# jrnerupudinho/Semi-Blind-Channel-Estimation-for-MIMO-RIS-communication-system-Using-EM-Algo

Measured on AMD Instinct MI355X. Metric: EM-iterations/sec (whole node) + NMSE@SNR; Nt=Nr=4, N_RIS=64, Tp=16 Td=256, higher is better.
Workload: dtype f64; 1 GPU; cfg1; n_tx=4, n_rx=4, N_RIS=64, T_p=16, T_d=256, M=16, trials_per_gpu=1000, em_iters=20, estep=soft, partition_r=0, solve=chol, parallelism=trials-sharded x1, streams_per_gpu=3

## Files before the change

semi-blind-channel-estimation-for-mimo-ris-communication-system-using-em-algo_amd/csrc/api.hip:

```cpp
#include <stdlib.h>
#include <string.h>

#include <atomic>
#include <initializer_list>
#include <mutex>
#include <vector>

#include "sbce_internal.h"

using namespace sbce;

namespace sbce {

#if SBCE_AB
DebugConfig g_debug;

namespace {
void read_debug_env(DebugConfig& c) {
    c = kDebugDefault;
    auto env = [](const char* n) { const char* v = getenv(n); return (v && v[0]) ? v : nullptr; };
    const char* v;
    if ((v = env("SBCE_ESTEP_IMPL"))) c.estep_valu = v[0] == 'v';
    if ((v = env("SBCE_ESTEP_PRUNE"))) c.estep_noprune = v[0] == '0';
    if ((v = env("SBCE_ESTEP_COUNT"))) c.estep_count = v[0] == '1';
    if ((v = env("SBCE_ESTEP_F32"))) c.estep_nof32 = v[0] == '0';
    if ((v = env("SBCE_ESTEP_SPHERE"))) c.estep_nosphere = v[0] == '0';
    if ((v = env("SBCE_SPHERE_BUDGET"))) {
        const int bu = atoi(v);
        c.sphere_budget = bu < 1 ? 1 : (bu > kBfsPmax ? kBfsPmax : bu);
    }
    if ((v = env("SBCE_BACKSUB"))) c.backsub_general = v[0] == '1';
    if ((v = env("SBCE_CHOL_IMPL"))) c.chol_valu = v[0] == 'v';
    if ((v = env("SBCE_ESTEP_PAIR"))) c.estep_nopair = v[0] == '0';
    if ((v = env("SBCE_CPLX3"))) c.cplx3 = v[0] != '0';
    if ((v = env("SBCE_MSTEP_SMALL"))) {
        c.mstep_nosmall = v[0] == '0';
        c.small_valu = v[0] == 'v';
        c.small_v1 = v[0] == '1';
    }
    if ((v = env("SBCE_PM_IMPL"))) c.pm_impl = (v[0] == 'w' || v[0] == 't' || v[0] == 'q') ? v[0] : 0;
    if ((v = env("SBCE_SMALL_SOLVE"))) c.small_col = v[0] == 'c';
    if ((v = env("SBCE_ESTEP_TRI"))) c.estep_tri = (v[0] >= '0' && v[0] <= '2') ? v[0] - '0' : 1;
    if ((v = env("SBCE_ESTEP_ORDER"))) c.estep_noorder = v[0] == '0';
    if ((v = env("SBCE_SMALL_STOP"))) c.small_stop = (v[0] >= '1' && v[0] <= '4') ? v[0] - '0' : 0;
}

__attribute__((constructor)) void load_debug_env() { read_debug_env(g_debug); }
}

bool debug_nondefault() {
    const DebugConfig& c = g_debug;
    const DebugConfig& d = kDebugDefault;
    return c.estep_valu != d.estep_valu || c.estep_noprune != d.estep_noprune ||
           c.estep_nof32 != d.estep_nof32 || c.estep_tri != d.estep_tri || c.estep_noorder != d.estep_noorder ||
           c.estep_nosphere != d.estep_nosphere || c.sphere_budget != d.sphere_budget ||
           c.backsub_general != d.backsub_general || c.chol_valu != d.chol_valu ||
           c.estep_nopair != d.estep_nopair || c.cplx3 != d.cplx3 ||
           c.mstep_nosmall != d.mstep_nosmall || c.small_stop != d.small_stop ||
           c.small_valu != d.small_valu || c.small_v1 != d.small_v1 || c.small_col != d.small_col ||
           (chol_debug_skip_mask() & 31);
}
#else
bool debug_nondefault() { return false; }
#endif

}

namespace {

constexpr size_t kAlign = 256;
size_t align_up(size_t v) { return (v + kAlign - 1) / kAlign * kAlign; }

struct Carve {
    size_t mom, R, rhs, done, mchg, ysh, prep, list, tree, tol, winv, ppsi, pS, pflag, prhs, gram, grhs,
        act, tol2, dvec, mnr, mnskip, total;
    bool has_prep, has_prhs, has_winv, has_mn;
};

constexpr int kAnySolve = -1;

bool make_problem(const sbce_dims* d, Problem& pb) {
    if (!d) return false;
    if (d->batch < 0 || d->n_tx < 1 || d->n_rx < 1 || d->n_psi < 1 || d->t_p < 0 || d->t_d < 1 ||
        d->m < 2 || d->partition_r < 0 || !(d->varn > 0.0))
        return false;
    if (d->n_tx > 8 || d->n_rx > 8) return false;
    pb.B = d->batch; pb.NT = d->n_tx; pb.NR = d->n_rx; pb.P = d->n_psi;
// ... 777 lines not shown
    Problem pb;
    if (!make_problem(d, pb) || !out3) return SBCE_EINVAL;
    int rc = check_ptrs(p, pb, true, SBCE_SOLVE_MINNORM);
    if (rc) return rc;
    if (pb.B == 0) return SBCE_OK;
    const Carve c = carve(pb, SBCE_SOLVE_MINNORM);
    MstepArgs ma;
    ma.R = (cd*)((char*)p->workspace + c.R);
    ma.done = nullptr;
    ma.nbatch = pb.B;
    set_large(ma, (char*)p->workspace, c);
    return hip_rc(launch_minnorm_rank(pb, ma, out3, (hipStream_t)hip_stream));
}

int sbce_debug_reload_env(void) {
#if SBCE_AB
    read_debug_env(g_debug);
    return debug_nondefault() ? 1 : 0;
#else
    return -1;
#endif
}

int sbce_debug_estep_mfma(unsigned long long* out, int reset) {
    if (!reset && !out) return SBCE_EINVAL;
    return hip_rc(estep_debug_mfma(out, reset));
}

int sbce_debug_estep_groups(unsigned long long* out, int reset) {
    if (!reset && !out) return SBCE_EINVAL;
    return hip_rc(estep_debug_groups(out, reset));
}

int sbce_debug_momskip(unsigned long long* out, int reset) {
#if SBCE_AB
    if (!reset && !out) return SBCE_EINVAL;
    return hip_rc(mstep_debug_momskip(out, reset));
#else
    (void)out; (void)reset;
    return SBCE_EUNSUPPORTED;
#endif
}

int sbce_debug_estep_sphere(unsigned long long* out3, int reset) {
    if (!reset && !out3) return SBCE_EINVAL;
    return hip_rc(estep_debug_sphere(out3, reset));
}

int sbce_debug_estep_pair(unsigned long long* out, int reset) {
    if (!reset && !out) return SBCE_EINVAL;
    return hip_rc(estep_debug_pair(out, reset));
}

int sbce_ser(const sbce_dims* d, const void* x_dest, const void* x_d_true, double* ser_out,
             void* hip_stream) {
    clear_stale_error();
    Problem pb;
    if (!make_problem(d, pb) || !x_dest || !x_d_true || !ser_out) return SBCE_EINVAL;
    if (pb.B == 0) return SBCE_OK;
    return hip_rc(launch_ser(pb, (const cd*)x_dest, (const cd*)x_d_true, ser_out,
                             (hipStream_t)hip_stream));
}

int sbce_gauss_expand(const sbce_dims* d, const void* theta, void* h_out, void* hip_stream) {
    clear_stale_error();
    Problem pb;
// ... 133 lines not shown
```

semi-blind-channel-estimation-for-mimo-ris-communication-system-using-em-algo_amd/csrc/estep_sweep.hip:

```cpp
#include "sbce_internal.h"

namespace sbce {

namespace {


template <int NT, int NR>
__device__ double candidate_distance(const cd* H, const cd* yg, const cd* s_cons, int M,
                                     double reg, cd* scratch, int lane, double& scale) {
    cd* sG = scratch;
    cd* sHy = scratch + 16;
    if (lane < NT * NT) {
        const int u = lane / NT, v = lane - u * NT;
        cd acc = czero();
#pragma unroll
        for (int r = 0; r < NR; ++r) acc = cfmac(acc, H[v * NR + r], H[u * NR + r]);
        if (u == v) acc.x += reg;
        sG[lane] = acc;
    } else if (lane >= 32 && lane < 32 + NT) {
        const int u = lane - 32;
        cd acc = czero();
#pragma unroll
        for (int r = 0; r < NR; ++r) acc = cfmac(acc, yg[r], H[u * NR + r]);
        sHy[u] = acc;
// ... 46 lines not shown
        const double od = shfl_xor_d(bd, off);
        const int os = __shfl_xor(bs, off);
        if (od < bd || (od == bd && os < bs)) { bd = od; bs = os; }
    }
    cd x[NT];
#pragma unroll
    for (int q = 0; q < NT; ++q) x[q] = s_cons[__shfl(bs, 16 * q)];
    double d0 = 0.0, sc = 0.0;
#pragma unroll
    for (int r = 0; r < NR; ++r) {
        cd res = yg[r];
        sc += cabs2(res);
#pragma unroll
        for (int q = 0; q < NT; ++q) {
            const cd hx = cmul(H[q * NR + r], x[q]);
            res = csub(res, hx);
            sc += NT * cabs2(hx);
        }
        d0 += cabs2(res);
    }
    wave_sync();
    scale = sc;
    return d0;
}


constexpr int kMfmaWaves = 2;
constexpr int kChunk = 256;
constexpr int kScreenD = 256;

typedef float f4v __attribute__((ext_vector_type(4)));

constexpr int mfma_rec_d(int rec_words) { return 2 * (rec_words <= 128 ? 160 : (rec_words + 1) / 2 * 2 + 32); }
constexpr int mfma_tri_d(int steps) { return 3 * 64 * steps / 2 + 128; }
constexpr int mfma_tab_d(int NO, int chunk, int steps, int M, int nkt_pad, int rec_words) {
    return (2 * NO + chunk + 3 * (4 * steps) * M + nkt_pad + 128 + 1) / 2 * 2 + mfma_rec_d(rec_words) +
           kScreenD + (M == 16 && chunk == 256 ? mfma_tri_d(steps) : 0);
}
constexpr int kTriGate = 4;

struct MfmaConst {
    int B, Td, P, M, lm;
    int JA, JB, chunk, nparts;
    int tab_d;
    double inv_s2, thr_d;
    double reg;
    int nkt_pad;
    int prune;
    int count;
    int prep_stride;
    int rowb_off;
    int rowb;
    int rec_words;
    int spw;
    int screen;
    int tri;
    int order;
};

template <int NT, int NR>
__device__ double column_tile_bounds(const cd* H, const cd* yg, const cd* s_cons, int M, int lm,
                                     int nkt, double* s_lb, cd* scratch, int lane) {
    constexpr int NA = NT / 2, NB = NT - NA;
    const int mask = M - 1;
    const int r = lane & 7;
    const bool own = r < NR;
    int xa[6];
#pragma unroll
    for (int i = 0; i < 6; ++i) xa[i] = (lane ^ (32 >> i)) << 2;
    auto rsum = [&](double v) {
#pragma unroll
        for (int i = 3; i < 6; ++i) v += bperm_d(v, xa[i]);
        return v;
    };
    auto rdot = [&](cd u, cd v) { return cmk(rsum(fma(v.x, u.x, v.y * u.y)),
                                             rsum(fma(v.y, u.x, -v.x * u.y))); };
    cd u[NA];
    bool ok = true;
#pragma unroll
    for (int q = 0; q < NA; ++q) {
        cd v = own ? H[q * NR + r] : czero();
        const double h2 = rsum(cabs2(v));
#pragma unroll
        for (int rep = 0; rep < 2; ++rep)
#pragma unroll
            for (int j = 0; j < q; ++j) v = csub(v, cmul(u[j], rdot(u[j], v)));
        const double n2 = rsum(cabs2(v));
        ok = ok && h2 > 0.0 && n2 > 1e-6 * h2;
        u[q] = cscale(v, ok ? fast_rsqrt(n2) : 0.0);
// ... 18 lines not shown
#pragma unroll
        for (int b = 0; b < NB; ++b) scratch[8 * (b + 1) + r] = g[b];
    }
    double cmax2 = lane < M ? cabs2(s_cons[lane]) : 0.0;
#pragma unroll
    for (int i = 0; i < 6; ++i) cmax2 = fmax(cmax2, bperm_d(cmax2, xa[i]));
    sc += NB * cmax2 * rsum(g2);
    wave_sync();
    for (int kt0 = 0; kt0 < nkt; kt0 += 4) {
        const int kt = kt0 + (lane >> 4);
        const int k = kt * 16 + (lane & 15);
        cd xb[NB];
#pragma unroll
        for (int b = 0; b < NB; ++b) xb[b] = s_cons[(k >> (lm * (NB - 1 - b))) & mask];
        double lb = 0.0;
#pragma unroll
        for (int rr = 0; rr < NR; ++rr) {
            cd res = scratch[rr];
#pragma unroll
            for (int b = 0; b < NB; ++b) res = csub(res, cmul(scratch[8 * (b + 1) + rr], xb[b]));
            lb += cabs2(res);
        }
        if (!ok) lb = 0.0;
#pragma unroll
        for (int i = 2; i < 6; ++i) lb = fmin(lb, bperm_d(lb, xa[i]));
        if ((lane & 15) == 0 && kt < nkt) s_lb[kt] = lb;
    }
    wave_sync();
    return sc;
}

__device__ unsigned long long g_estep_mfma;
__device__ unsigned long long g_estep_groups;

template <int NT, int NR, int MODE, int TU, bool V16>
__device__ __forceinline__ void estep_mfma_body(const EstepArgs& a, const MfmaConst& c) {
    static_assert(!V16 || NT == 4, "the V16 body is the n_tx = 4, M = 16 sweep");
    const int k_M = V16 ? 16 : c.M;
    const int k_lm = V16 ? 4 : c.lm;
    const int k_JA = V16 ? 256 : c.JA;
    const int k_JB = V16 ? 256 : c.JB;
    const int k_chunk = V16 ? 256 : c.chunk;
    const int k_nkt_pad = V16 ? 16 : c.nkt_pad;
    const int k_rowb_off = V16 ? 4 + 2 * NT * NR + 16 : c.rowb_off;
    const int k_prep_stride = V16 ? k_rowb_off + 6 * NR : c.prep_stride;
    const int k_rec_words = V16 ? k_prep_stride + 2 * NR : c.rec_words;
    const int k_tab_d = V16 ? mfma_tab_d(NT * NR, 256, (2 * NR + 3) / 4, 16, 16, k_rec_words) : c.tab_d;
    constexpr int NA = NT / 2;
    constexpr int NB = NT - NA;
    constexpr int NO = NT * NR;
    constexpr int K2 = 2 * NR;
    constexpr int STEPS = (K2 + 3) / 4;
    constexpr int NPA = NA * (NA - 1) / 2;
    constexpr int NPB = NB * (NB - 1) / 2;
    static_assert(NA >= 1 && NA <= 2 && NB <= 2, "mfma E-step: 2 <= n_tx <= 4");

    if (a.list && (long)blockIdx.x * kMfmaWaves >= (long)a.list[(long)c.B * c.Td]) return;
    extern __shared__ __attribute__((aligned(16))) char smem[];
    cd* s_cons = reinterpret_cast<cd*>(smem);
    const int wave = __builtin_amdgcn_readfirstlane(threadIdx.x >> 6);
    const int lane = threadIdx.x & 63;
    double* wbase = reinterpret_cast<double*>(s_cons + 64) + (size_t)wave * k_tab_d;
    cd* s_heff = reinterpret_cast<cd*>(wbase);
    double* s_al = wbase + 2 * NO;
    double* s_U = s_al + k_chunk;
    double* s_V = s_U + 4 * STEPS * k_M;
    double* s_Q2 = s_V + 4 * STEPS * k_M;
    double* s_lb = s_Q2 + 4 * STEPS * k_M;
    double* s_tab = s_lb + k_nkt_pad;
    double* s_recb = s_tab + 128;
    float* s_al32 = reinterpret_cast<float*>(s_recb + mfma_rec_d(k_rec_words));
    float* s_U32 = s_al32 + 256;

    for (int i = threadIdx.x; i < k_M; i += blockDim.x) s_cons[i] = a.cons[i];
    __syncthreads();

    const long nsym = (long)c.B * c.Td;
    const bool listed = a.list != nullptr;
    int32_t* cnt = listed ? a.list + nsym : nullptr;
    const long nwork = listed ? (long)__builtin_amdgcn_readfirstlane(cnt[0]) : nsym;
    const bool prep = a.prep != nullptr;
    auto sym_of = [&](long gi) -> long { return listed ? (long)a.list[gi] : gi; };
    bool first = true;
    for (;;) {
    long chunk_id;
    if (listed) {
        if (first) {
            chunk_id = (long)blockIdx.x * kMfmaWaves + wave;
        } else {
            int v = 0;
            if (lane == 0) v = atomicAdd(cnt + 1, 1);
            chunk_id = (long)gridDim.x * kMfmaWaves + __builtin_amdgcn_readfirstlane(__shfl(v, 0));
        }
        first = false;
    } else {
        chunk_id = (long)blockIdx.x * kMfmaWaves + wave;
    }
    const int spw = listed ? 1 : c.spw;
    const long g0 = chunk_id * spw;
    if (g0 >= nwork) return;
    const long g1 = g0 + spw < nwork ? g0 + spw : nwork;
    const bool dma = prep && k_rec_words <= 128;
    auto issue = [&](long g, double* dst) {
        int l = lane;
        asm volatile("" : "+v"(l));
        const int hs = k_prep_stride >> 1;
        const double* src = a.prep + (size_t)g * k_prep_stride;
        if (l < hs) src += 2 * l;
        else if (l < (k_rec_words >> 1))
            src = reinterpret_cast<const double*>(a.yd) + (size_t)g * 2 * NR + 2 * (l - hs);
        __builtin_amdgcn_global_load_lds((const __attribute__((address_space(1))) void*)src,
                                         (__attribute__((address_space(3))) void*)dst, 16, 0, 0);
        if (a.done)
            __builtin_amdgcn_global_load_lds(
                (const __attribute__((address_space(1))) void*)(a.done + g / c.Td),
                (__attribute__((address_space(3))) void*)(dst + 128), 4, 0, 0);
    };
    if (dma) issue(sym_of(g0), s_recb);
    for (long gi = g0; gi < g1; ++gi) {
    const long gsym = sym_of(gi);
    const int cur = (int)((gi - g0) & 1);
    double* s_rec = s_recb + cur * 160;
    int dn;
    if (dma) {
        asm volatile("s_waitcnt vmcnt(0)" ::: "memory");
        wave_sync();
        dn = a.done ? reinterpret_cast<const int*>(s_rec + 128)[0] : 0;
        if (gi + 1 < g1) issue(sym_of(gi + 1), s_recb + (cur ^ 1) * 160);
    } else {
        dn = a.done ? a.done[gsym / c.Td] : 0;
        if (prep && !dn) {
            wave_sync();
            for (int e = lane; e < k_rec_words; e += 64)
                s_rec[e] = e < k_prep_stride
                    ? a.prep[(size_t)gsym * k_prep_stride + e]
                    : reinterpret_cast<const double*>(a.yd)[(size_t)gsym * 2 * NR + e - k_prep_stride];
            wave_sync();
        }
    }
    if (dn) continue;
    int lane_s = lane;
    asm volatile("" : "+v"(lane_s));
    [&, lane = lane_s]() {
    const int b = (int)(gsym / c.Td);
    const int t = (int)(gsym - (long)b * c.Td);
    const int mask = k_M - 1;
    double thr_d = c.thr_d, inv_s2 = c.inv_s2, reg = c.reg;
    if (a.varn_t) {
        const TrialNoise tn = trial_noise(a.varn_t[b]);
        thr_d = uniform_d(tn.thr_d);
        inv_s2 = uniform_d(tn.inv_s2);
        reg = uniform_d(tn.reg);
    }

    if (prep) {
    } else {
        const cd* th = a.theta + (size_t)b * c.P * NO;
        const cd* ps = a.psid + (size_t)gsym * c.P;
        const int ntask = NO * c.nparts;
        cd* part = reinterpret_cast<cd*>(s_tab);
        if (lane < ntask) {
// ... 205 lines not shown
#pragma unroll
            for (int j = 0; j < 4; ++j) {
                const double us = bperm_d(uu, (4 * rq + j) << 2);
                tA[(4 * rq + j) * 16 + col] = (float)fma(0.5, (double)cx[j], 0.25 * (us + vv));
            }
            wave_sync();
            double tq = 0.0;
#pragma unroll 1
            for (int blk = 0; blk < 4; ++blk) {
                f4v t[4];
#pragma unroll
                for (int u = 0; u < 4; ++u)
                    t[u] = *reinterpret_cast<const f4v*>(tA + (4 * blk + u) * 16 + rq * 4);
#pragma unroll
                for (int s = 0; s < STEPS; ++s)
#pragma unroll
                    for (int u = 0; u < 4; ++u)
                        t[u] = __builtin_amdgcn_mfma_f32_16x16x4f32(
                            tU[(4 * s + rq) * 16 + 4 * blk + u] + vr32[s], qr32[s], t[u], 0, 0, 0);
                float mm = fminf(fminf(t[0][0], t[0][1]), fminf(t[0][2], t[0][3]));
#pragma unroll
                for (int u = 1; u < 4; ++u)
                    mm = fminf(mm, fminf(fminf(t[u][0], t[u][1]), fminf(t[u][2], t[u][3])));
                mm = fminf(mm, __int_as_float(__builtin_amdgcn_ds_bpermute(xaddr16, __float_as_int(mm))));
                mm = fminf(mm, __int_as_float(__builtin_amdgcn_ds_bpermute(xaddr32, __float_as_int(mm))));
                if (rq == blk) tq = ((double)mm + qq) - margin;
            }
            tri_lane = fmax(tri_lane, tq);
        }
    };

    const double hard_bound = d0 + 1e-10 * cscale_d + 1e-300;
    unsigned groups = 0;
    unsigned reached = 0;
    constexpr bool ORD = V16 && MODE != SBCE_ESTEP_HARD;
    const bool ordered = ORD && (SBCE_AB ? c.order != 0 : true);
    unsigned long long ktord = 0xfedcba9876543210ull;
    if constexpr (ORD) {
        if (ordered) {
            const double lbc = lbp[col];
            const double mine = lbc < lb_margin ? 0.0 : lbc;
            int rank = 0;
#pragma unroll
            for (int j = 0; j < 16; ++j) {
                const double lbj = lbp[j];
                const double o = lbj < lb_margin ? 0.0 : lbj;
                rank += (o < mine || (o == mine && j < col)) ? 1 : 0;
            }
            const unsigned nib = (unsigned)col << ((rank & 7) << 2);
            unsigned lo = rank < 8 ? nib : 0u, hi = rank < 8 ? 0u : nib;
            auto row_or = [](unsigned v) {
                v |= (unsigned)__builtin_amdgcn_update_dpp(0, (int)v, 0xB1, 0xF, 0xF, false);
                v |= (unsigned)__builtin_amdgcn_update_dpp(0, (int)v, 0x4E, 0xF, 0xF, false);
                v |= (unsigned)__builtin_amdgcn_update_dpp(0, (int)v, 0x141, 0xF, 0xF, false);
                v |= (unsigned)__builtin_amdgcn_update_dpp(0, (int)v, 0x140, 0xF, 0xF, false);
                return (unsigned)__builtin_amdgcn_readfirstlane((int)v);
            };
            lo = row_or(lo);
            hi = row_or(hi);
            ktord = ((unsigned long long)hi << 32) | lo;
        }
    }
    [[maybe_unused]] unsigned long long ktmask = ~0ull;
    if (!ORD && nktile <= 64) {
        const double lim0 = ((MODE == SBCE_ESTEP_HARD) ? hard_bound : mshift + thr_d) + lb_margin;
        ktmask = __ballot(lane < nktile && !(lbp[lane < nktile ? lane : 0] > lim0));
// ... 198 lines not shown
                    if (V16) {
                        const cd lo = *reinterpret_cast<const cd*>(s_al + (tg + u) * 16 + rq * 4);
                        const cd hi = *reinterpret_cast<const cd*>(s_al + (tg + u) * 16 + rq * 4 + 2);
                        acc[u] = mf4{lo.x, lo.y, hi.x, hi.y};
                    } else {
#pragma unroll
                        for (int j = 0; j < 4; ++j) acc[u][j] = s_al[(tg + u) * 16 + rq + 4 * j];
                    }
                }
#pragma unroll
                for (int s = 0; s < STEPS; ++s)
#pragma unroll
                    for (int u = 0; u < TU; ++u) {
                        const int kk = 4 * s + rq;
                        double av;
                        if (V16) {
                            av = s_U[kk * 16 + (i0 >> 4) + tg + u] + vreg[s];
                        } else {
                            const int ia = i0 + (tg + u) * 16 + col;
                            av = s_U[kk * k_M + ((NA == 2) ? (ia >> k_lm) : ia)];
                            if (NA == 2) av += s_V[kk * k_M + (ia & mask)];
                        }
                        acc[u] = __builtin_amdgcn_mfma_f64_16x16x4f64(av, bop[s], acc[u], 0, 0, 0);
                    }
                double cm = fmin(fmin(acc[0][0], acc[0][1]), fmin(acc[0][2], acc[0][3]));
#pragma unroll
                for (int u = 1; u < TU; ++u)
                    cm = fmin(cm, fmin(fmin(acc[u][0], acc[u][1]), fmin(acc[u][2], acc[u][3])));
                if (MODE == SBCE_ESTEP_HARD) {
                    if (!__any(cm + gam <= best_d)) continue;
                } else if (!__any(cm + gam <= mshift + thr_d)) {
                    continue;
                }
                if (MODE == SBCE_ESTEP_HARD) {
                    const double lim = best_d - gam;
#pragma unroll
                    for (int u = 0; u < TU; ++u)
#pragma unroll
                        for (int j = 0; j < 4; ++j) {
                            const double dv = acc[u][j];
                            if (dv <= lim) {
                                const int jj = (i0 + (tg + u) * 16 + rq + 4 * j) * k_JB + k;
                                const double dd = dv + gam;
                                if (dd < best_d || (dd == best_d && jj < best_j)) { best_d = dd; best_j = jj; }
                            }
                        }
                    continue;
                }
                cm += gam;
                if (__any(cm < mshift)) {
                    double mn = fmin(cm, mshift);
                    mn = wave_min_dpp(mn);
                    const double f = fexp_neg((mn - mshift) * inv_s2);
                    mshift = mn;
                    constexpr int NBS = V16 ? 1 : NB;
                    tot_c *= f; kap = cscale(kap, f);
                    if constexpr (!V16) { ck *= f; tot_kB = cscale(tot_kB, f); }
#pragma unroll
                    for (int q = 0; q < NA; ++q) {
                        tot_muA[q] = cscale(tot_muA[q], f); nu[q] *= f;
                        if constexpr (!V16) mu[q] = cscale(mu[q], f);
#pragma unroll
                        for (int bb = 0; bb < NBS; ++bb) tot_X[q][bb] = cscale(tot_X[q][bb], f);
                    }
#pragma unroll
                    for (int bb = 0; bb < NBS; ++bb) { tot_mB[bb] = cscale(tot_mB[bb], f); tot_nB[bb] *= f; }
// ... 12 lines not shown
                    if (!__any(cmu <= mshift + thr_d)) continue;
                    if constexpr (V16) {
                        const cd x0 = s_cons[tg + u];
                        const double n0 = cabs2(x0);
#pragma unroll
                        for (int j = 0; j < 4; ++j) {
                            const double dj = acc[u][j] + gam;
                            if (!__any(dj <= mshift + thr_d)) continue;
                            const double w = fexp_neg((mshift - dj) * inv_s2);
                            R1[j] += w;
                            Q[j] = caxpy(Q[j], w, x0);
                            N0 = fma(w, n0, N0);
                        }
                        continue;
                    }
#pragma unroll
                    for (int j = 0; j < 4; ++j) {
                        const int i = i0 + (tg + u) * 16 + rq + 4 * j;
                        const double w = fexp_neg((mshift - (acc[u][j] + gam)) * inv_s2);
                        cd xa[NA];
#pragma unroll
                        for (int q = 0; q < NA; ++q) xa[q] = s_cons[(i >> (k_lm * (NA - 1 - q))) & mask];
                        ck += w;
#pragma unroll
                        for (int q = 0; q < NA; ++q) {
                            mu[q] = caxpy(mu[q], w, xa[q]);
                            nu[q] = fma(w, cabs2(xa[q]), nu[q]);
                        }
                        if (NPA) kap = caxpy(kap, w, cmulc(xa[0], xa[NA > 1 ? 1 : 0]));
                    }
                }
            }
        }
        if (MODE == SBCE_ESTEP_SOFT && touched) {
            if constexpr (V16) {
                ck = (R1[0] + R1[1]) + (R1[2] + R1[3]);
                mu[0] = cadd(cadd(Q[0], Q[1]), cadd(Q[2], Q[3]));
                mu[1] = czero();
                nu[0] += N0;
#pragma unroll
                for (int j = 0; j < 4; ++j) {
                    const cd x1 = s_cons[rq + 4 * j];
                    mu[1] = caxpy(mu[1], R1[j], x1);
                    nu[1] = fma(R1[j], cabs2(x1), nu[1]);
                    kap = cadd(kap, cmulc(Q[j], x1));
                }
            }
            constexpr int NBS = V16 ? 1 : NB;
            tot_c += ck;
#pragma unroll
            for (int bb = 0; bb < NBS; ++bb) {
                tot_mB[bb] = caxpy(tot_mB[bb], ck, xb[bb]);
                tot_nB[bb] = fma(ck, cabs2(xb[bb]), tot_nB[bb]);
            }
            if (NPB && !V16) tot_kB = caxpy(tot_kB, ck, cmulc(xb[0], xb[NB > 1 ? 1 : 0]));
#pragma unroll
            for (int q = 0; q < NA; ++q) {
                tot_muA[q] = cadd(tot_muA[q], mu[q]);
#pragma unroll
                for (int bb = 0; bb < NBS; ++bb) tot_X[q][bb] = cfmac(tot_X[q][bb], mu[q], xb[bb]);
            }
        }
    }
    if constexpr (V16) {
        const cd x3 = s_cons[col];
        tot_mB[1] = cscale(x3, tot_c);
        tot_nB[1] = tot_c * cabs2(x3);
        tot_kB = cmulc(tot_mB[0], x3);
#pragma unroll
        for (int q = 0; q < NA; ++q) tot_X[q][1] = cmulc(tot_muA[q], x3);
    }

    if (c.count && lane == 0) {
        atomicAdd(&g_estep_mfma, (unsigned long long)groups * STEPS * TU);
        if (V16) atomicAdd(&g_estep_groups, (unsigned long long)reached);
    }
    constexpr int MS = NT + NT * NT;
    cd* out = a.mom + (size_t)gsym * MS;
    const bool arm = a.mchg != nullptr;
    cd mold = czero();
    if (arm && lane < MS) mold = out[lane];
    if (MODE == SBCE_ESTEP_HARD) {
        wave_argmin_dpp(best_d, best_j);
        if (lane < MS) {
            const int s2 = lane < NT ? lane : (lane - NT) / NT;
            const int s3 = lane < NT ? 0 : (lane - NT) % NT;
            const cd xp = s_cons[(best_j >> (k_lm * (NT - 1 - s2))) & mask];
            const cd xq = s_cons[(best_j >> (k_lm * (NT - 1 - s3))) & mask];
            const cd mv = mom_word(lane < NT ? xp : cmulc(xp, xq));
            out[lane] = mv;
            if (arm && mom_bits_differ(mold, mv)) a.mchg[b] = 1;
        }
        return;
    }
    int xa[6];
#pragma unroll
    for (int i = 0; i < 6; ++i) xa[i] = (lane ^ (32 >> i)) << 2;
    {
        constexpr int NV = 1 + 2 * NPA + 2 * NPB + 3 * NA + 2 * NA * NB + 3 * NB;
        static_assert(NV <= 32, "reduce-scatter holds at most 32 values");
        double v[32];
        int n = 0;
        auto put = [&](double x) { v[n++] = x; };
        put(tot_c);
        if (NPA) { put(kap.x); put(kap.y); }
        if (NPB) { put(tot_kB.x); put(tot_kB.y); }
#pragma unroll
        for (int q = 0; q < NA; ++q) {
// ... 33 lines not shown
                ire = lane < NA ? BQ + lane * SQ : BB + 3 * (lane - NA);
                iim = ire + 1;
            } else {
                const int i = (lane - NT) / NT, j = (lane - NT) - (lane - NT) / NT * NT;
                if (i == j) {
                    ire = i < NA ? BQ + i * SQ + 2 : BB + 3 * (i - NA) + 2;
                } else if (i < NA && j < NA) {
                    ire = OFF_KA; iim = OFF_KA + 1; cj = i > j;
                } else if (i >= NA && j >= NA) {
                    ire = OFF_KB; iim = OFF_KB + 1; cj = i > j;
                } else if (i < NA) {
                    ire = BQ + i * SQ + 3 + 2 * (j - NA); iim = ire + 1;
                } else {
                    ire = BQ + j * SQ + 3 + 2 * (i - NA); iim = ire + 1; cj = true;
                }
            }
            const double iz = 1.0 / red[0];
            const double re = red[ire], im = iim >= 0 ? red[iim] : 0.0;
            const cd mv = mom_word(cmk(re * iz, (cj ? -im : im) * iz));
            out[lane] = mv;
            if (arm && mom_bits_differ(mold, mv)) a.mchg[b] = 1;
        }
    }
    }();
    }
    if (!listed) return;
    }
}

template <int NT, int NR, int MODE, int TU, bool V16 = false>
__global__ __launch_bounds__(128) void estep_mfma_kernel(EstepArgs a, MfmaConst c) {
    estep_mfma_body<NT, NR, MODE, TU, V16>(a, c);
}
bool make_mfma(const Problem& pb, MfmaConst& c, size_t& lds, long& blocks) {
    HypSplit h;
    if (!hyp_split(pb, h) || h.JA < 16 || h.JB < 16) return false;
    const long JA = h.JA, JB = h.JB;
    c.B = pb.B; c.Td = pb.Td; c.P = pb.P; c.M = pb.M; c.lm = h.lm;
    c.JA = (int)JA; c.JB = (int)JB;
    c.chunk = (int)(JA < kChunk ? JA : kChunk);
    const int NO = pb.NT * pb.NR;
    c.nparts = NO <= 64 ? 64 / NO : 1;
    const int steps = (2 * pb.NR + 3) / 4;
    c.nkt_pad = (int)((JB / 16 + 1) / 2 * 2);

    c.prune = !g_debug.estep_noprune;
    c.count = g_debug.estep_count;
    c.inv_s2 = 1.0 / (pb.varn * pb.varn);
    c.thr_d = kSkipThr * pb.varn * pb.varn;
    c.reg = 0.1 * pb.varn * pb.varn;
    c.rowb_off = 4 + 2 * NO + c.nkt_pad;
    c.prep_stride = c.rowb_off + (pb.NT == 4 ? 6 * pb.NR : 0);
    c.rec_words = c.prep_stride + 2 * pb.NR;
    c.tab_d = mfma_tab_d(NO, c.chunk, steps, pb.M, c.nkt_pad, c.rec_words);
    c.spw = 4;
    c.screen = !g_debug.estep_nof32;
    c.tri = g_debug.estep_tri;
    c.order = !g_debug.estep_noorder;
    c.rowb = pb.NT == 4 && c.prune;
    lds = 64 * sizeof(cd) + (size_t)kMfmaWaves * c.tab_d * sizeof(double);
    const long nsym = (long)pb.B * pb.Td;
    const long per_block = (long)kMfmaWaves * c.spw;
    blocks = (nsym + per_block - 1) / per_block;
    return lds <= 160 * 1024;
}

template <int NT, int NR>
hipError_t dispatch_mfma_mode(const MfmaConst& c, size_t lds, long blocks, const EstepArgs& a,
                              int mode, hipStream_t s) {
    const bool tu4 = (c.chunk / 16) % 4 == 0;
    if constexpr (NT == 4) {
        if (c.M == 16 && tu4) {
            if (c.JA != 256 || c.JB != 256 || c.chunk != 256 || c.nkt_pad != 16 ||
                c.prep_stride != 4 + 2 * NT * NR + 16 + 6 * NR)
                return hipErrorInvalidValue;
            if (mode == SBCE_ESTEP_HARD)
                hipLaunchKernelGGL((estep_mfma_kernel<NT, NR, SBCE_ESTEP_HARD, 4, true>),
                                   dim3((unsigned)blocks), dim3(64 * kMfmaWaves), lds, s, a, c);
            else
                hipLaunchKernelGGL((estep_mfma_kernel<NT, NR, SBCE_ESTEP_SOFT, 4, true>),
                                   dim3((unsigned)blocks), dim3(64 * kMfmaWaves), lds, s, a, c);
            return hipGetLastError();
        }
    }
    if (mode == SBCE_ESTEP_HARD) {
        if (tu4)
            hipLaunchKernelGGL((estep_mfma_kernel<NT, NR, SBCE_ESTEP_HARD, 4>), dim3((unsigned)blocks),
                               dim3(64 * kMfmaWaves), lds, s, a, c);
        else
            hipLaunchKernelGGL((estep_mfma_kernel<NT, NR, SBCE_ESTEP_HARD, 1>), dim3((unsigned)blocks),
                               dim3(64 * kMfmaWaves), lds, s, a, c);
    } else {
        if (tu4)
            hipLaunchKernelGGL((estep_mfma_kernel<NT, NR, SBCE_ESTEP_SOFT, 4>), dim3((unsigned)blocks),
                               dim3(64 * kMfmaWaves), lds, s, a, c);
        else
            hipLaunchKernelGGL((estep_mfma_kernel<NT, NR, SBCE_ESTEP_SOFT, 1>), dim3((unsigned)blocks),
                               dim3(64 * kMfmaWaves), lds, s, a, c);
    }
    return hipGetLastError();
}

template <int NT>
hipError_t dispatch_mfma_nr(int NR, const MfmaConst& c, size_t lds, long blocks,
                            const EstepArgs& a, int mode, hipStream_t s) {
    switch (NR) {
        case 1: return dispatch_mfma_mode<NT, 1>(c, lds, blocks, a, mode, s);
        case 2: return dispatch_mfma_mode<NT, 2>(c, lds, blocks, a, mode, s);
        case 3: return dispatch_mfma_mode<NT, 3>(c, lds, blocks, a, mode, s);
        case 4: return dispatch_mfma_mode<NT, 4>(c, lds, blocks, a, mode, s);
        case 5: return dispatch_mfma_mode<NT, 5>(c, lds, blocks, a, mode, s);
        case 6: return dispatch_mfma_mode<NT, 6>(c, lds, blocks, a, mode, s);
        case 7: return dispatch_mfma_mode<NT, 7>(c, lds, blocks, a, mode, s);
        case 8: return dispatch_mfma_mode<NT, 8>(c, lds, blocks, a, mode, s);
    }
    return hipErrorInvalidValue;
}

}

hipError_t estep_debug_mfma(unsigned long long* out, int reset) {
    if (reset) {
        const unsigned long long z = 0;
        return hipMemcpyToSymbol(HIP_SYMBOL(g_estep_mfma), &z, sizeof(z), 0, hipMemcpyHostToDevice);
    }
    return hipMemcpyFromSymbol(out, HIP_SYMBOL(g_estep_mfma), sizeof(*out), 0,
                               hipMemcpyDeviceToHost);
}

hipError_t estep_debug_groups(unsigned long long* out, int reset) {
    if (reset) {
        const unsigned long long z = 0;
        return hipMemcpyToSymbol(HIP_SYMBOL(g_estep_groups), &z, sizeof(z), 0, hipMemcpyHostToDevice);
    }
    return hipMemcpyFromSymbol(out, HIP_SYMBOL(g_estep_groups), sizeof(*out), 0,
                               hipMemcpyDeviceToHost);
}

SweepPlan estep_sweep_plan(const Problem& pb) {
    MfmaConst c;
    size_t lds;
    long blocks;
    if (!make_mfma(pb, c, lds, blocks)) return SweepPlan{};
    return SweepPlan{true, c.lm, c.JB, c.prep_stride, c.count, c.reg, c.inv_s2, c.thr_d, blocks};
}

int estep_prep_stride(const Problem& pb) { return estep_sweep_plan(pb).prep_stride; }

hipError_t launch_estep_sweep(const Problem& pb, const EstepArgs& a, int mode, long blocks,
                              hipStream_t s) {
    MfmaConst c;
    size_t lds;
    long all;
    if (!make_mfma(pb, c, lds, all)) return hipErrorInvalidValue;
    switch (pb.NT) {
        case 2: return dispatch_mfma_nr<2>(pb.NR, c, lds, blocks, a, mode, s);
        case 3: return dispatch_mfma_nr<3>(pb.NR, c, lds, blocks, a, mode, s);
        case 4: return dispatch_mfma_nr<4>(pb.NR, c, lds, blocks, a, mode, s);
    }
    return hipErrorInvalidValue;
}

// ... 2 lines not shown
```

semi-blind-channel-estimation-for-mimo-ris-communication-system-using-em-algo_amd/csrc/sbce_internal.h:

```cpp
#pragma once

#include <hip/hip_runtime.h>
#include <stdint.h>
#include <math.h>

#include "../../include/sbce.h"

namespace sbce {

typedef double2 cd;

typedef double mf4 __attribute__((ext_vector_type(4)));
__device__ __forceinline__ mf4 mfma4(double a, double b, mf4 c) {
    return __builtin_amdgcn_mfma_f64_16x16x4f64(a, b, c, 0, 0, 0);
}
template <bool G3>
__device__ __forceinline__ void csub_init(mf4& cre, mf4& cim, mf4& c2) {
    c2 = mf4{0.0, 0.0, 0.0, 0.0};
    if constexpr (G3) cim += cre;
}
template <bool G3>
__device__ __forceinline__ void csub_step(mf4& cre, mf4& cim, mf4& c2, cd v, cd t) {
    if constexpr (G3) {
        cre = __builtin_amdgcn_mfma_f64_16x16x4f64(-v.x, t.x, cre, 0, 0, 0);
// ... 154 lines not shown
    return __builtin_amdgcn_ldexp(y, -h);
}
__device__ __forceinline__ double fast_rsqrt64(double x) {
    double y = __builtin_amdgcn_rsq(x);
    double r = fma(-x * y, y, 1.0);
    y = fma(0.5 * y, r, y);
    r = fma(-x * y, y, 1.0);
    return fma(0.5 * y, r, y);
}


#ifndef SBCE_AB
#define SBCE_AB 0
#endif
struct DebugConfig {
    bool estep_valu;
    bool estep_noprune;
    bool estep_count;
    bool estep_nof32;
    bool estep_nosphere;
    int sphere_budget;
    bool backsub_general;
    bool chol_valu;
    bool estep_nopair;
    bool cplx3;
    bool mstep_nosmall;
    bool small_valu;
    bool small_v1;
    int small_stop;
    bool small_col;
    char pm_impl;
    int estep_tri;
    bool estep_noorder;
};
inline constexpr DebugConfig kDebugDefault = {false, false, false, false, false, 128, false, false,
                                              false, true, false, false, false, 0, false, 0, 1, false};
#if SBCE_AB
extern DebugConfig g_debug;
#else
inline constexpr DebugConfig g_debug = kDebugDefault;
#endif
bool debug_nondefault();

struct Problem {
    int B, NT, NR, P, Tp, Td, M, L, K;
    int pr;
    double varn;
    double varx;
};

struct EstepArgs {
    const cd* yd;
    const cd* psid;
    const cd* theta;
    const cd* cons;
    cd* mom;
    const int32_t* done;
    int32_t* status;
    double* prep;
    int32_t* list;
    double* tree;
    const double* varn_t = nullptr;
    bool lists_zeroed = false;
    int32_t* mchg = nullptr;
};

__device__ __forceinline__ unsigned mom_bits_differ(const cd& u, const cd& v) {
    const unsigned long long d = ((unsigned long long)__double_as_longlong(u.x) ^
                                  (unsigned long long)__double_as_longlong(v.x)) |
// ... 182 lines not shown
hipError_t launch_mstep_small(const Problem& pb, const MstepArgs& a, bool write_sys, hipStream_t s);
int chol_debug_skip_mask();
constexpr int kLargeL = 512;
constexpr int kMaxL = 8192;
bool rbuild_herm_supported(const Problem& pb);
hipError_t chol_debug_timing(int mode, double* out6);
hipError_t launch_pilot_factor(const Problem& pb, const MstepArgs& a, hipStream_t s);
hipError_t launch_rbuild_herm(const Problem& pb, const MstepArgs& a, hipStream_t s);
hipError_t launch_chol_large(const Problem& pb, const MstepArgs& a, hipStream_t s);
hipError_t launch_diag_tol(const Problem& pb, const MstepArgs& a, hipStream_t s);
hipError_t launch_chol_tile(const Problem& pb, const MstepArgs& a, int k0, int w, const int32_t* ext,
                            hipStream_t s);
hipError_t launch_tile_factor_step(const Problem& pb, const MstepArgs& a, int k, const TileExt& e,
                                   hipStream_t s);
hipError_t launch_tile_factor(const Problem& pb, const MstepArgs& a, const TileExt& e,
                              hipError_t (*act_check)(const Problem&, const MstepArgs&, int, hipStream_t),
                              hipStream_t s);
hipError_t launch_minnorm_rank(const Problem& pb, const MstepArgs& a, int32_t* out, hipStream_t s);
hipError_t launch_tile_back(const Problem& pb, const MstepArgs& a, const int32_t* ext, hipStream_t s);
hipError_t launch_minnorm(const Problem& pb, const MstepArgs& a, hipStream_t s);
hipError_t chol_debug_clock(unsigned long long* out);
hipError_t chol_debug_clock_reset();
void chol_debug_skip(int mask);
int chol_debug_skip_mask();
hipError_t launch_decisions(const Problem& pb, const cd* mom, cd* xdest, hipStream_t s);
hipError_t launch_sup_shift_y(const Problem& pb, const cd* yd, const cd* psid, const cd* theta,
                              const cd* xsup, cd* yout, const int32_t* done, hipStream_t s);
hipError_t launch_sup_shift_mom(const Problem& pb, cd* mom, const cd* xsup, const int32_t* done,
                                hipStream_t s);
hipError_t launch_ser(const Problem& pb, const cd* xdest, const cd* xtrue, double* out,
                      hipStream_t s);
hipError_t estep_debug_mfma(unsigned long long* out, int reset);
hipError_t estep_debug_groups(unsigned long long* out, int reset);
bool estep_momfold_supported(const Problem& pb, int mode);
hipError_t mstep_debug_momskip(unsigned long long* out, int reset);
hipError_t estep_debug_sphere(unsigned long long* out3, int reset);
bool estep_pair_supported(const Problem& pb, int mode);
hipError_t launch_estep_pair(const Problem& pb, const EstepArgs& a, int stride, int count, int mode,
                             hipStream_t s);
hipError_t estep_debug_pair(unsigned long long* out, int reset);
hipError_t launch_gauss_rank1(const Problem& pb, const MstepArgs& a, hipStream_t s);
hipError_t launch_gauss_expand(const Problem& pb, const cd* theta, cd* out, hipStream_t s);
hipError_t launch_nmse(const Problem& pb, const cd* theta, const cd* h, double* out,
                       hipStream_t s);
hipError_t launch_llf(const Problem& pb, const cd* theta, const cd* yp, const cd* up,
                      const cd* yd, const cd* psid, const cd* xd, double* llf, int iters,
                      int it, const int32_t* done, const double* varn_t, hipStream_t s);
hipError_t launch_em_init(int B, int32_t* done, int32_t* mchg, int32_t* status, int status_value, int32_t* cnt,
                          hipStream_t s, FreezeReport* rep = nullptr, int32_t gen = 0,
                          int32_t* word = nullptr);
hipError_t launch_early_stop(const Problem& pb, const cd* theta, const cd* h,
                             int32_t* done, int32_t* iters_done, int it, hipStream_t s);

struct ApproxArgs {
    const cd* yd;
    const cd* yp;
    const cd* psid;
    const cd* psip;
    const cd* xp;
    cd* g;
    const double* varn_t;
    int32_t* status;
    int B, N, M, Tp, Td, iters;
    double varn;
    int status0;
};
// ... 122 lines not shown
```

Before: 1.527 million EM-iterations/s.

## Split V16 soft E-step into bound pass then exact soft-weight pass

Adds a two-pass variant of the V16 soft E-step sweep. The first pass only computes the running minimum distance and records which (kt, tile) blocks pass the threshold in a 64-bit hit mask. The second pass revisits only the marked blocks to accumulate soft weights against the final minimum. This avoids accumulating against a moving shift and lets the record double buffer shrink LDS use when a worklist is present. The cost is recomputing MFMA products for the hit blocks and extra branch logic.

```diff
diff --git a/semi-blind-channel-estimation-for-mimo-ris-communication-system-using-em-algo_amd/csrc/api.hip b/semi-blind-channel-estimation-for-mimo-ris-communication-system-using-em-algo_amd/csrc/api.hip
--- a/semi-blind-channel-estimation-for-mimo-ris-communication-system-using-em-algo_amd/csrc/api.hip
+++ b/semi-blind-channel-estimation-for-mimo-ris-communication-system-using-em-algo_amd/csrc/api.hip
@@ -42,6 +42,7 @@
     if ((v = env("SBCE_SMALL_SOLVE"))) c.small_col = v[0] == 'c';
     if ((v = env("SBCE_ESTEP_TRI"))) c.estep_tri = (v[0] >= '0' && v[0] <= '2') ? v[0] - '0' : 1;
     if ((v = env("SBCE_ESTEP_ORDER"))) c.estep_noorder = v[0] == '0';
+    if ((v = env("SBCE_ESTEP_TWOPASS"))) c.estep_notwopass = v[0] == '0';
     if ((v = env("SBCE_SMALL_STOP"))) c.small_stop = (v[0] >= '1' && v[0] <= '4') ? v[0] - '0' : 0;
 }
 
@@ -53,6 +54,7 @@
     const DebugConfig& d = kDebugDefault;
     return c.estep_valu != d.estep_valu || c.estep_noprune != d.estep_noprune ||
            c.estep_nof32 != d.estep_nof32 || c.estep_tri != d.estep_tri || c.estep_noorder != d.estep_noorder ||
+           c.estep_notwopass != d.estep_notwopass ||
            c.estep_nosphere != d.estep_nosphere || c.sphere_budget != d.sphere_budget ||
            c.backsub_general != d.backsub_general || c.chol_valu != d.chol_valu ||
            c.estep_nopair != d.estep_nopair || c.cplx3 != d.cplx3 ||
@@ -896,6 +898,11 @@
     return hip_rc(estep_debug_groups(out, reset));
 }
 
+int sbce_debug_estep_pass2(unsigned long long* out, int reset) {
+    if (!reset && !out) return SBCE_EINVAL;
+    return hip_rc(estep_debug_pass2(out, reset));
+}
+
 int sbce_debug_momskip(unsigned long long* out, int reset) {
 #if SBCE_AB
     if (!reset && !out) return SBCE_EINVAL;
diff --git a/semi-blind-channel-estimation-for-mimo-ris-communication-system-using-em-algo_amd/csrc/estep_sweep.hip b/semi-blind-channel-estimation-for-mimo-ris-communication-system-using-em-algo_amd/csrc/estep_sweep.hip
--- a/semi-blind-channel-estimation-for-mimo-ris-communication-system-using-em-algo_amd/csrc/estep_sweep.hip
+++ b/semi-blind-channel-estimation-for-mimo-ris-communication-system-using-em-algo_amd/csrc/estep_sweep.hip
@@ -102,6 +102,7 @@
 typedef float f4v __attribute__((ext_vector_type(4)));
 
 constexpr int mfma_rec_d(int rec_words) { return 2 * (rec_words <= 128 ? 160 : (rec_words + 1) / 2 * 2 + 32); }
+constexpr int mfma_rec_half_v16(int NT, int NR) { return mfma_rec_d(4 + 2 * NT * NR + 16 + 8 * NR) / 2; }
 constexpr int mfma_tri_d(int steps) { return 3 * 64 * steps / 2 + 128; }
 constexpr int mfma_tab_d(int NO, int chunk, int steps, int M, int nkt_pad, int rec_words) {
     return (2 * NO + chunk + 3 * (4 * steps) * M + nkt_pad + 128 + 1) / 2 * 2 + mfma_rec_d(rec_words) +
@@ -125,6 +126,7 @@
     int spw;
     int screen;
     int tri;
+    int twopass;
     int order;
 };
 
@@ -209,10 +211,12 @@
 
 __device__ unsigned long long g_estep_mfma;
 __device__ unsigned long long g_estep_groups;
-
-template <int NT, int NR, int MODE, int TU, bool V16>
+__device__ unsigned long long g_estep_pass2;
+
+template <int NT, int NR, int MODE, int TU, bool V16, bool TP = false, bool REC = false>
 __device__ __forceinline__ void estep_mfma_body(const EstepArgs& a, const MfmaConst& c) {
     static_assert(!V16 || NT == 4, "the V16 body is the n_tx = 4, M = 16 sweep");
+    static_assert(!TP || (V16 && MODE == SBCE_ESTEP_SOFT && TU == 4), "two-pass: the V16 soft sweep");
     const int k_M = V16 ? 16 : c.M;
     const int k_lm = V16 ? 4 : c.lm;
     const int k_JA = V16 ? 256 : c.JA;
@@ -222,7 +226,9 @@
     const int k_rowb_off = V16 ? 4 + 2 * NT * NR + 16 : c.rowb_off;
     const int k_prep_stride = V16 ? k_rowb_off + 6 * NR : c.prep_stride;
     const int k_rec_words = V16 ? k_prep_stride + 2 * NR : c.rec_words;
-    const int k_tab_d = V16 ? mfma_tab_d(NT * NR, 256, (2 * NR + 3) / 4, 16, 16, k_rec_words) : c.tab_d;
+    constexpr int REC_H = mfma_rec_half_v16(NT, NR);
+    const int k_tab_d = V16 ? mfma_tab_d(NT * NR, 256, (2 * NR + 3) / 4, 16, 16, k_rec_words) - (TP ? REC_H : 0)
+                            : c.tab_d;
     constexpr int NA = NT / 2;
     constexpr int NB = NT - NA;
     constexpr int NO = NT * NR;
@@ -246,7 +252,13 @@
     double* s_lb = s_Q2 + 4 * STEPS * k_M;
     double* s_tab = s_lb + k_nkt_pad;
     double* s_recb = s_tab + 128;
-    float* s_al32 = reinterpret_cast<float*>(s_recb + mfma_rec_d(k_rec_words));
+    float* s_al32 = reinterpret_cast<float*>(s_recb + (TP ? REC_H : mfma_rec_d(k_rec_words)));
+    [[maybe_unused]] double* s_rec2 =
+        reinterpret_cast<double*>(s_cons + 64) + (size_t)kMfmaWaves * k_tab_d + (size_t)wave * REC_H;
+    auto rec_half = [&](int h) -> double* {
+        if constexpr (TP) return h ? s_rec2 : s_recb;
+        else return s_recb + h * 160;
+    };
     float* s_U32 = s_al32 + 256;
 
     for (int i = threadIdx.x; i < k_M; i += blockDim.x) s_cons[i] = a.cons[i];
@@ -256,7 +268,7 @@
     const bool listed = a.list != nullptr;
     int32_t* cnt = listed ? a.list + nsym : nullptr;
     const long nwork = listed ? (long)__builtin_amdgcn_readfirstlane(cnt[0]) : nsym;
-    const bool prep = a.prep != nullptr;
+    const bool prep = REC || a.prep != nullptr;
     auto sym_of = [&](long gi) -> long { return listed ? (long)a.list[gi] : gi; };
     bool first = true;
     for (;;) {
@@ -297,13 +309,13 @@
     for (long gi = g0; gi < g1; ++gi) {
     const long gsym = sym_of(gi);
     const int cur = (int)((gi - g0) & 1);
-    double* s_rec = s_recb + cur * 160;
+    double* s_rec = rec_half(cur);
     int dn;
     if (dma) {
         asm volatile("s_waitcnt vmcnt(0)" ::: "memory");
         wave_sync();
         dn = a.done ? reinterpret_cast<const int*>(s_rec + 128)[0] : 0;
-        if (gi + 1 < g1) issue(sym_of(gi + 1), s_recb + (cur ^ 1) * 160);
+        if (gi + 1 < g1) issue(sym_of(gi + 1), rec_half(cur ^ 1));
     } else {
         dn = a.done ? a.done[gsym / c.Td] : 0;
         if (prep && !dn) {
@@ -575,6 +587,7 @@
 
     const double hard_bound = d0 + 1e-10 * cscale_d + 1e-300;
     unsigned groups = 0;
+    [[maybe_unused]] unsigned long long hit = 0;
     unsigned reached = 0;
     constexpr bool ORD = V16 && MODE != SBCE_ESTEP_HARD;
     const bool ordered = ORD && (SBCE_AB ? c.order != 0 : true);
@@ -839,6 +852,12 @@
                 } else if (!__any(cm + gam <= mshift + thr_d)) {
                     continue;
                 }
+                if constexpr (TP) {
+                    cm += gam;
+                    if (__any(cm < mshift)) mshift = wave_min_dpp(fmin(cm, mshift));
+                    hit |= 1ull << (4 * kt + (tg >> 2));
+                    continue;
+                }
                 if (MODE == SBCE_ESTEP_HARD) {
                     const double lim = best_d - gam;
 #pragma unroll
@@ -917,7 +936,7 @@
                 }
             }
         }
-        if (MODE == SBCE_ESTEP_SOFT && touched) {
+        if (!TP && MODE == SBCE_ESTEP_SOFT && touched) {
             if constexpr (V16) {
                 ck = (R1[0] + R1[1]) + (R1[2] + R1[3]);
                 mu[0] = cadd(cadd(Q[0], Q[1]), cadd(Q[2], Q[3]));
@@ -947,6 +966,74 @@
             }
         }
     }
+    [[maybe_unused]] unsigned groups2 = 0;
+    if constexpr (TP) {
+        for (unsigned long long left = hit; left;) {
+            const int kt = __builtin_ctzll(left) >> 2;
+            const unsigned blks = (unsigned)(left >> (4 * kt)) & 15u;
+            left &= ~(15ull << (4 * kt));
+            double bop[STEPS];
+            double gam = 0.0;
+#pragma unroll
+            for (int s = 0; s < STEPS; ++s) {
+                bop[s] = s_Q2[(4 * s + rq) * 16 + kt] + q3reg[s];
+                gam = fma(bop[s], bop[s], gam);
+            }
+            gam += bperm_d(gam, xaddr16);
+            gam += bperm_d(gam, xaddr32);
+            double R1[4] = {0.0, 0.0, 0.0, 0.0}, N0 = 0.0;
+            cd Q[4] = {czero(), czero(), czero(), czero()};
+            bool touched = false;
+            groups2 += __builtin_popcount(blks);
+#pragma unroll 1
+            for (int tl = 0; tl < 16; ++tl) {
+                if (!((blks >> (tl >> 2)) & 1u)) continue;
+                const cd lo = *reinterpret_cast<const cd*>(s_al + tl * 16 + rq * 4);
+                const cd hi = *reinterpret_cast<const cd*>(s_al + tl * 16 + rq * 4 + 2);
+                mf4 acc = mf4{lo.x, lo.y, hi.x, hi.y};
+#pragma unroll
+                for (int s = 0; s < STEPS; ++s)
+                    acc = __builtin_amdgcn_mfma_f64_16x16x4f64(s_U[(4 * s + rq) * 16 + tl] + vreg[s], bop[s],
+                                                               acc, 0, 0, 0);
+                const double cmu = fmin(fmin(acc[0], acc[1]), fmin(acc[2], acc[3])) + gam;
+                if (!__any(cmu <= mshift + thr_d)) continue;
+                touched = true;
+                const cd x0 = s_cons[tl];
+                const double n0 = cabs2(x0);
+#pragma unroll
+                for (int j = 0; j < 4; ++j) {
+                    const double dj = acc[j] + gam;
+                    if (!__any(dj <= mshift + thr_d)) continue;
+                    const double w = fexp_neg((mshift - dj) * inv_s2);
+                    R1[j] += w;
+                    Q[j] = caxpy(Q[j], w, x0);
+                    N0 = fma(w, n0, N0);
+                }
+            }
+            if (!touched) continue;
+            const cd x2 = s_cons[kt];
+            const double ck = (R1[0] + R1[1]) + (R1[2] + R1[3]);
+            cd mu[NA];
+            mu[0] = cadd(cadd(Q[0], Q[1]), cadd(Q[2], Q[3]));
+            mu[1] = czero();
+            nu[0] += N0;
+#pragma unroll
+            for (int j = 0; j < 4; ++j) {
+                const cd x1 = s_cons[rq + 4 * j];
+                mu[1] = caxpy(mu[1], R1[j], x1);
+                nu[1] = fma(R1[j], cabs2(x1), nu[1]);
+                kap = cadd(kap, cmulc(Q[j], x1));
+            }
+            tot_c += ck;
+            tot_mB[0] = caxpy(tot_mB[0], ck, x2);
+            tot_nB[0] = fma(ck, cabs2(x2), tot_nB[0]);
+#pragma unroll
+            for (int q = 0; q < NA; ++q) {
+                tot_muA[q] = cadd(tot_muA[q], mu[q]);
+                tot_X[q][0] = cfmac(tot_X[q][0], mu[q], x2);
+            }
+        }
+    }
     if constexpr (V16) {
         const cd x3 = s_cons[col];
         tot_mB[1] = cscale(x3, tot_c);
@@ -959,6 +1046,7 @@
     if (c.count && lane == 0) {
         atomicAdd(&g_estep_mfma, (unsigned long long)groups * STEPS * TU);
         if (V16) atomicAdd(&g_estep_groups, (unsigned long long)reached);
+        if (TP) atomicAdd(&g_estep_pass2, (unsigned long long)groups2);
     }
     constexpr int MS = NT + NT * NT;
     cd* out = a.mom + (size_t)gsym * MS;
@@ -1058,6 +1146,10 @@
 __global__ __launch_bounds__(128) void estep_mfma_kernel(EstepArgs a, MfmaConst c) {
     estep_mfma_body<NT, NR, MODE, TU, V16>(a, c);
 }
+template <int NR, bool REC>
+__global__ __launch_bounds__(128) void estep_twopass_kernel(EstepArgs a, MfmaConst c) {
+    estep_mfma_body<4, NR, SBCE_ESTEP_SOFT, 4, true, true, REC>(a, c);
+}
 bool make_mfma(const Problem& pb, MfmaConst& c, size_t& lds, long& blocks) {
     HypSplit h;
     if (!hyp_split(pb, h) || h.JA < 16 || h.JB < 16) return false;
@@ -1083,6 +1175,7 @@
     c.screen = !g_debug.estep_nof32;
     c.tri = g_debug.estep_tri;
     c.order = !g_debug.estep_noorder;
+    c.twopass = !g_debug.estep_notwopass;
     c.rowb = pb.NT == 4 && c.prune;
     lds = 64 * sizeof(cd) + (size_t)kMfmaWaves * c.tab_d * sizeof(double);
     const long nsym = (long)pb.B * pb.Td;
@@ -1100,12 +1193,25 @@
             if (c.JA != 256 || c.JB != 256 || c.chunk != 256 || c.nkt_pad != 16 ||
                 c.prep_stride != 4 + 2 * NT * NR + 16 + 6 * NR)
                 return hipErrorInvalidValue;
-            if (mode == SBCE_ESTEP_HARD)
+            if (mode == SBCE_ESTEP_HARD) {
                 hipLaunchKernelGGL((estep_mfma_kernel<NT, NR, SBCE_ESTEP_HARD, 4, true>),
                                    dim3((unsigned)blocks), dim3(64 * kMfmaWaves), lds, s, a, c);
+                return hipGetLastError();
+            }
+            if constexpr (SBCE_AB) {
+                if (!c.twopass) {
+                    hipLaunchKernelGGL((estep_mfma_kernel<NT, NR, SBCE_ESTEP_SOFT, 4, true>),
+                                       dim3((unsigned)blocks), dim3(64 * kMfmaWaves), lds, s, a, c);
+                    return hipGetLastError();
+                }
+            }
+            const size_t lds2 = a.list ? lds - kMfmaWaves * mfma_rec_half_v16(NT, NR) * sizeof(double) : lds;
+            if (a.prep)
+                hipLaunchKernelGGL((estep_twopass_kernel<NR, true>), dim3((unsigned)blocks),
+                                   dim3(64 * kMfmaWaves), lds2, s, a, c);
             else
-                hipLaunchKernelGGL((estep_mfma_kernel<NT, NR, SBCE_ESTEP_SOFT, 4, true>),
-                                   dim3((unsigned)blocks), dim3(64 * kMfmaWaves), lds, s, a, c);
+                hipLaunchKernelGGL((estep_twopass_kernel<NR, false>), dim3((unsigned)blocks),
+                                   dim3(64 * kMfmaWaves), lds2, s, a, c);
             return hipGetLastError();
         }
     }
@@ -1154,6 +1260,15 @@
                                hipMemcpyDeviceToHost);
 }
 
+hipError_t estep_debug_pass2(unsigned long long* out, int reset) {
+    if (reset) {
+        const unsigned long long z = 0;
+        return hipMemcpyToSymbol(HIP_SYMBOL(g_estep_pass2), &z, sizeof(z), 0, hipMemcpyHostToDevice);
+    }
+    return hipMemcpyFromSymbol(out, HIP_SYMBOL(g_estep_pass2), sizeof(*out), 0,
+                               hipMemcpyDeviceToHost);
+}
+
 hipError_t estep_debug_groups(unsigned long long* out, int reset) {
     if (reset) {
         const unsigned long long z = 0;
diff --git a/semi-blind-channel-estimation-for-mimo-ris-communication-system-using-em-algo_amd/csrc/sbce_internal.h b/semi-blind-channel-estimation-for-mimo-ris-communication-system-using-em-algo_amd/csrc/sbce_internal.h
--- a/semi-blind-channel-estimation-for-mimo-ris-communication-system-using-em-algo_amd/csrc/sbce_internal.h
+++ b/semi-blind-channel-estimation-for-mimo-ris-communication-system-using-em-algo_amd/csrc/sbce_internal.h
@@ -210,9 +210,10 @@
     char pm_impl;
     int estep_tri;
     bool estep_noorder;
+    bool estep_notwopass;
 };
 inline constexpr DebugConfig kDebugDefault = {false, false, false, false, false, 128, false, false,
-                                              false, true, false, false, false, 0, false, 0, 1, false};
+                                              false, true, false, false, false, 0, false, 0, 1, false, false};
 #if SBCE_AB
 extern DebugConfig g_debug;
 #else
@@ -461,6 +462,7 @@
                       hipStream_t s);
 hipError_t estep_debug_mfma(unsigned long long* out, int reset);
 hipError_t estep_debug_groups(unsigned long long* out, int reset);
+hipError_t estep_debug_pass2(unsigned long long* out, int reset);
 bool estep_momfold_supported(const Problem& pb, int mode);
 hipError_t mstep_debug_momskip(unsigned long long* out, int reset);
 hipError_t estep_debug_sphere(unsigned long long* out3, int reset);
```

New measurement: 1.605 million EM-iterations/s (median of 6 runs). +5.1%, better.
